# SMSD75/Timetuning

Hardware: AMD Instinct MI355X
Metric: clip-frames/sec (higher is better)
Workload: dtype f32-split(f16x3); 1 GPU; C2: dino-s16 full TimeT training step (fwd+bwd+AdamW), 4-frame 224x224 clips, 32 clips/GPU, 200 prototypes; clips_per_gpu=32, num_frames=4, num_clusters=200, global_batch=32, parallelism=dp1

## Files before the change

include/timetuning_hip.h:

```cpp
#ifndef TIMETUNING_HIP_H
#define TIMETUNING_HIP_H

#include <stddef.h>
#include <stdint.h>

#ifdef __cplusplus
extern "C" {
#endif

#define TT_OK 0
#define TT_EINVAL (-1)
#define TT_ELAUNCH (-2)
#define TT_EUNSUPPORTED (-3)

typedef void* tt_stream_t;

const char* tt_last_error(void);
int tt_abi_version(void);
int tt_set_tuning_knob(const char* name, int value);
int tt_tuning_knob_info(int index, const char** name, int* default_value, int* value);
int tt_device_info(char* name, int cap);

size_t tt_linear_ksplit_workspace_bytes(void);
int tt_linear_ksplit_workspace_init(void* workspace, size_t workspace_bytes, tt_stream_t stream);
// ... 130 lines not shown
int tt_linear_bwd_weight_planes(const void* dyT_planes, long long dyT_plane_stride, const void* xT_planes, long long xT_plane_stride,
                                int planes, float* dw, int N, int K, int Mpad, void* workspace, size_t workspace_bytes,
                                tt_stream_t stream);
size_t tt_linear_bwd_weight_planes_workspace_bytes(int N, int K, int Mpad);

int tt_label_propagate_route(int fs, int g, int K, int n_last_frames, int radius, int t);
int tt_label_propagate(const float* xn, const float* seg0, int64_t* labels, double* pmap_last, int bs, int fs, int g,
                       int D, int K, int n_last_frames, int radius, int topk, float temperature, int precision, void* workspace,
                       size_t workspace_bytes, tt_stream_t stream);
size_t tt_label_propagate_workspace_bytes(int bs, int fs, int g, int D, int K, int n_last_frames);
int tt_label_propagate_sims(const float* xn, int bs, int fs, int g, int D, int K, int n_last_frames, int precision, void* workspace,
                            size_t workspace_bytes, tt_stream_t stream);
int tt_label_propagate_from_sims(const float* xn, const float* seg0, int64_t* labels, double* pmap_last, int bs, int fs, int g, int D, int K,
                                 int n_last_frames, int radius, int topk, float temperature, void* workspace, size_t workspace_bytes,
                                 tt_stream_t stream);

int tt_label_propagate_maps(const float* xn, const float* seg0, double* pmap_all, int bs, int fs, int g, int D, int K,
                            int n_last_frames, int radius, int topk, float temperature, int precision, void* workspace,
                            size_t workspace_bytes, tt_stream_t stream);
int tt_upsample_argmax(const double* maps, int64_t* labels_out, int M, int g, int K, int R, tt_stream_t stream);
int tt_confusion_counts(const int64_t* pred, const int64_t* gt, long long n, int C, unsigned long long* counts,
                        tt_stream_t stream);

#define TT_LABELS_I16 0
#define TT_LABELS_I64 1
int tt_confusion_segments_route(int Cg, int Cp);
int tt_confusion_counts_segments(const void* pred, int pred_dtype, const int64_t* gt, int S, long long n, int Cg, int Cp, long long ignore_gt,
                                 int has_ignore, unsigned long long* counts, tt_stream_t stream);

#define TT_LABELS_U8 2
// ... 174 lines not shown
```

timetuning_amd/_lib.py:

```python
from __future__ import annotations

import ctypes as C
import os
import subprocess

_HERE = os.path.dirname(os.path.abspath(__file__))
LIB_PATH = os.environ.get("TT_LIB_PATH") or os.path.join(_HERE, "libtimetuning_hip.so")
CSRC = os.path.join(_HERE, "csrc")

c_f32p = C.c_void_p
c_vp = C.c_void_p
c_i = C.c_int
c_ll = C.c_longlong
c_f = C.c_float
c_d = C.c_double
c_sz = C.c_size_t


class AdamwTensor(C.Structure):
    _fields_ = [("p", C.c_void_p), ("g", C.c_void_p), ("m", C.c_void_p), ("v", C.c_void_p), ("n", C.c_longlong),
                ("lr", C.c_float), ("weight_decay", C.c_float)]


class VitBlockParams(C.Structure):
# ... 125 lines not shown
    "tt_kmeans_assign_route": (c_i, [c_i]),
    "tt_kmeans_accumulate": (c_i, [c_vp, c_vp, c_vp, c_vp, c_ll, c_i, c_i, c_vp, c_sz, c_vp]),
    "tt_kmeans_tiled_shape_ok": (c_i, [c_i, c_i]),
    "tt_kmeans_tile_centroids": (c_i, [c_i]),
    "tt_kmeans_assign_tiled": (c_i, [c_vp, c_vp, c_vp, c_vp, c_ll, c_i, c_i, c_i, c_vp]),
    "tt_kmeans_accumulate_tiled_workspace_bytes": (c_sz, [c_ll, c_i, c_i, c_i]),
    "tt_kmeans_accumulate_tiled": (c_i, [c_vp, c_vp, c_vp, c_vp, c_ll, c_i, c_i, c_i, c_vp, c_sz, c_vp]),
    "tt_kmeans_fit_shape_ok": (c_i, [c_ll, c_i, c_i]),
    "tt_kmeans_fit_lds_bytes": (c_sz, [c_ll, c_i, c_i]),
    "tt_kmeans_fit_workspace_bytes": (c_sz, [c_i, c_i, c_ll, c_i, c_i]),
    "tt_kmeans_fit_batched": (c_i, [c_vp, c_vp, c_vp, c_vp, c_vp, c_vp, c_i, c_ll, c_i, c_i, c_i, c_i, c_vp, c_sz, c_vp]),
    "tt_kmeans_fit_batched_split": (c_i, [c_vp, c_vp, c_vp, c_vp, c_vp, c_vp, c_i, c_ll, c_i, c_i, c_i, c_i, c_vp, c_sz, c_vp, c_i, c_vp]),
    "tt_kmeans_assign_batched": (c_i, [c_vp, c_vp, c_vp, c_vp, c_i, c_ll, c_i, c_i, c_vp]),
    "tt_label_propagate_sims": (c_i, [c_vp, c_i, c_i, c_i, c_i, c_i, c_i, c_i, c_vp, c_sz, c_vp]),
    "tt_label_propagate_from_sims": (c_i, [c_vp, c_vp, c_vp, c_vp, c_i, c_i, c_i, c_i, c_i, c_i, c_i, c_i, c_f, c_vp, c_sz, c_vp]),
    "tt_label_propagate_maps": (c_i, [c_vp, c_vp, c_vp, c_i, c_i, c_i, c_i, c_i, c_i, c_i, c_i, c_f, c_i, c_vp, c_sz, c_vp]),
    "tt_upsample_argmax": (c_i, [c_vp, c_vp, c_i, c_i, c_i, c_i, c_vp]),
    "tt_confusion_counts": (c_i, [c_vp, c_vp, c_ll, c_i, c_vp, c_vp]),
    "tt_confusion_segments_route": (c_i, [c_i, c_i]),
    "tt_confusion_counts_segments": (c_i, [c_vp, c_i, c_vp, c_i, c_ll, c_i, c_i, c_ll, c_i, c_vp, c_vp]),
    "tt_overlay_grid": (c_i, [c_vp, c_i, c_vp, C.POINTER(C.c_float), C.POINTER(C.c_float), c_vp, c_vp, c_i, c_i, c_i, c_vp, c_vp, c_vp, c_i, c_i, c_vp,
                              c_i, c_d, c_i, c_i, c_i, c_i, c_vp]),
    "tt_upsample_argmax_hist_f32": (c_i, [c_vp, c_vp, c_i, c_i, c_i, c_i, c_vp]),
    "tt_label_propagate_grid_workspace_bytes": (c_sz, [c_i, c_i, c_i, c_i, c_i, c_i, c_i, c_i]),
    "tt_label_propagate_grid_maps": (c_i, [c_vp, c_vp, c_vp, c_i, c_i, c_i, c_i, c_i, c_i, c_i, c_i, c_i, c_f, c_i, c_vp, c_sz, c_vp]),
    "tt_upsample_argmax_hw": (c_i, [c_vp, c_vp, c_i, c_i, c_i, c_i, c_i, c_i, c_vp]),
    "tt_probe_logits": (c_i, [c_vp, c_vp, c_vp, c_vp, c_ll, c_i, c_i, c_vp]),
    "tt_probe_upsample_ce_workspace_bytes": (c_sz, [c_i, c_i]),
    "tt_probe_upsample_ce": (c_i, [c_vp, c_vp, c_vp, c_vp, c_vp, c_i, c_i, c_i, c_i, c_vp, c_sz, c_vp]),
    "tt_bilinear_adjoint_tokens": (c_i, [c_vp, c_vp, c_i, c_i, c_i, c_i, c_vp]),
# ... 65 lines not shown
```

timetuning_amd/csrc/label_prop.hip:

```cpp
#include "common.hpp"

namespace tt {

int launch_gemm_plain2(const float* A, const float* B, float* C, int M, int N, int K, int lda, int ldb, int ldc, int batch_inner,
                       int batch_outer, long long sA, long long sB, long long sC, long long sA2, long long sB2, long long sC2, int bf16,
                       hipStream_t s);

constexpr int LP_MAXC = 8;
constexpr int LP_CAND_MAX = 16;

struct LpArgs {
  const float* sims;
  const float* seg0;
  const double* seg_prev;
  double* seg_out;
  int64_t* labels;
  int ctx_frame[LP_MAXC];
  int c, cs, bs, g, K, radius, topk;
  float temp;
};

template <int LP_CAND>
__global__ __launch_bounds__(256) void label_prop_kernel(LpArgs a) {
  __shared__ float s_val[4];
// ... 145 lines not shown
    s_besti[wave] = besti;
  }
  __syncthreads();
  if (tid == 0) {
    best = s_best[0];
    besti = s_besti[0];
    for (int w = 1; w < 4; ++w)
      if (s_best[w] > best || (s_best[w] == best && s_besti[w] < besti)) {
        best = s_best[w];
        besti = s_besti[w];
      }
    a.labels[(long long)b * n + qi] = besti;
  }
}

template <int CTX, int KT>
__global__ __launch_bounds__(256) void label_prop_wave_kernel(LpArgs a) {
  constexpr int CPL = 4 * CTX;
  const int lane = threadIdx.x & 63;
  const int n = a.g * a.g;
  const long long item = (long long)blockIdx.x * 4 + (threadIdx.x >> 6);
  if (item >= (long long)a.bs * n) return;
  const int b = (int)(item / n), qi = (int)(item - (long long)b * n);
  const int qy = qi / a.g, qx = qi - qy * a.g;
  const int y0 = max(0, qy - a.radius), y1 = min(a.g - 1, qy + a.radius);
  const int x0 = max(0, qx - a.radius), x1 = min(a.g - 1, qx + a.radius);
  const int ww = x1 - x0 + 1, wh = y1 - y0 + 1;
  const int total = ww * wh * a.c;
  const int lx = lane & 15, ly = lane >> 4;

  float val[CPL];
  int src[CPL];
#pragma unroll
  for (int j = 0; j < CTX; ++j) {
    const float* row = a.sims + (((long long)b * a.cs + j) * n + qi) * n;
#pragma unroll
    for (int r = 0; r < 4; ++r) {
      const int i = j * 4 + r, y = ly + 4 * r;
      val[i] = -1.f;
      src[i] = -1;
      if (j < a.c && lx < ww && y < wh) {
        const int sp = (y0 + y) * a.g + x0 + lx;
        val[i] = expf(row[sp] / a.temp);
        src[i] = (j << 12) | sp;
      }
    }
  }
  float thr = 0.f;
  unsigned taken = 0u;
  const int rounds = min(a.topk, total);
  for (int rd = 0; rd < rounds; ++rd) {
    float bv = -2.f;
    int bi = 0x7fffffff;
#pragma unroll
    for (int i = 0; i < CPL; ++i)
      if (!((taken >> i) & 1u) && src[i] >= 0 && val[i] > bv) {
        bv = val[i];
        bi = lane + 64 * i;
      }
#pragma unroll
    for (int o = 32; o > 0; o >>= 1) {
      const float ov = __shfl_xor(bv, o, 64);
      const int oi = __shfl_xor(bi, o, 64);
      if (ov > bv || (ov == bv && oi < bi)) {
        bv = ov;
        bi = oi;
      }
    }
    thr = bv;
    if ((bi & 63) == lane) taken |= 1u << (bi >> 6);
  }
  if (total < a.topk) thr = 0.f;
  float mysum = 0.f;
#pragma unroll
  for (int i = 0; i < CPL; ++i)
    if (src[i] >= 0 && val[i] >= thr) mysum += val[i];
  const float colsum = wave_sum(mysum);

  double acc[KT];
#pragma unroll
  for (int t = 0; t < KT; ++t) acc[t] = 0.0;
  const long long fstride = (long long)a.bs * n * a.K;
#pragma unroll
  for (int i = 0; i < CPL; ++i) {
    unsigned long long mask = __ballot(src[i] >= 0 && val[i] >= thr);
    while (mask) {
      const int l = __builtin_ctzll(mask);
      mask &= mask - 1;
      const int s_ = __shfl(src[i], l, 64);
      const double w = (double)(__shfl(val[i], l, 64) / colsum);
      const int fr = a.ctx_frame[s_ >> 12];
      const long long off = ((long long)b * n + (s_ & 4095)) * a.K;
#pragma unroll
      for (int t = 0; t < KT; ++t) {
        const int k = lane + 64 * t;
        if (k < a.K) acc[t] += ((fr == 0) ? (double)a.seg0[off + k] : a.seg_prev[(long long)(fr - 1) * fstride + off + k]) * w;
      }
    }
  }
  double best = -1.0;
  int besti = 0x7fffffff;
#pragma unroll
  for (int t = 0; t < KT; ++t) {
    const int k = lane + 64 * t;
    if (k < a.K) {
      a.seg_out[((long long)b * n + qi) * a.K + k] = acc[t];
      if (acc[t] > best) {
        best = acc[t];
        besti = k;
      }
    }
  }
  if (!a.labels) return;
#pragma unroll
  for (int o = 32; o > 0; o >>= 1) {
    const double ov = __shfl_xor(best, o, 64);
    const int oi = __shfl_xor(besti, o, 64);
    if (ov > best || (ov == best && oi < besti)) {
      best = ov;
      besti = oi;
    }
  }
  if (lane == 0) a.labels[(long long)b * n + qi] = besti;
}

__global__ void f64_copy_kernel(const double* __restrict__ src, double* __restrict__ dst, long long n) {
  long long i = (long long)blockIdx.x * blockDim.x + threadIdx.x;
  const long long st = (long long)gridDim.x * blockDim.x;
  for (; i < n; i += st) dst[i] = src[i];
}

static int lp_cmax(int fs, int n_last) {
  int c = 1 + (fs - 2 < n_last ? fs - 2 : n_last);
  return c < 1 ? 1 : c;
}

static int lp_route(int fs, int g, int K, int n_last, int radius, int t) {
  if (fs < 2 || g <= 0 || K <= 0 || n_last < 0 || n_last + 1 > LP_MAXC || radius <= 0 || t < 1 || t >= fs) return 0;
// ... 49 lines not shown

using namespace tt;

extern "C" size_t tt_label_propagate_workspace_bytes(int bs, int fs, int g, int D, int K, int n_last_frames) {
  (void)D;
  const size_t n = (size_t)g * g;
  return lp_workspace(lp_chunk(bs, fs, (int)n, n_last_frames), bs, fs, n, K, n_last_frames);
}

extern "C" int tt_label_propagate_route(int fs, int g, int K, int n_last_frames, int radius, int t) {
  return lp_route(fs, g, K, n_last_frames, radius, t);
}

static int lp_run(const char* who, const float* xn, const float* seg0, int64_t* labels, double* pmap_last, double* pmap_all, int bs,
                  int fs, int g, int D, int K, int n_last_frames, int radius, int topk, float temperature, int precision, void* workspace,
                  size_t workspace_bytes, tt_stream_t stream, int phase = 0) {
  TT_REQUIRE(xn && (seg0 || phase == 1) && workspace, "%s: null pointer", who);
  TT_REQUIRE(precision >= TT_PRECISION_F32 && precision <= TT_PRECISION_BF16, "%s: precision must be 0, 1 or 2 (got %d)", who, precision);
  const int sims_bf16 = precision == TT_PRECISION_BF16;
  TT_REQUIRE(bs > 0 && fs >= 2 && g > 0 && D > 0 && K > 0, "%s: need fs >= 2 and positive sizes", who);
  TT_REQUIRE(n_last_frames >= 0 && n_last_frames + 1 <= LP_MAXC, "%s: n_last_frames must be <= %d", who, LP_MAXC - 1);
  TT_REQUIRE(radius > 0, "%s: size_mask_neighborhood must be > 0 (the unrestricted variant is not built)", who);
  TT_REQUIRE(topk >= 1, "%s: topk >= 1", who);
  const int win = (2 * radius + 1 < g ? 2 * radius + 1 : g);
  const long long cand_max = (long long)win * win * lp_cmax(fs, n_last_frames);
  TT_REQUIRE(cand_max <= 256LL * LP_CAND_MAX, "%s: window %dx%d with %d context frames exceeds %d candidates per query", who, win, win,
             lp_cmax(fs, n_last_frames), 256 * LP_CAND_MAX);
  TT_REQUIRE(D % 4 == 0, "%s: feature dim must be a multiple of 4", who);
  if (lp_route(fs, g, K, n_last_frames, radius, 1) >= 5)
    TT_REQUIRE(bs <= 65535, "%s: %d clips exceed the 65535 of one launch of the workgroup-per-query kernel", who, bs);
  TT_REQUIRE(bs <= 65535, "%s: %d clips exceed the 65535 problems of one similarity launch", who, bs);
  hipStream_t s = as_stream(stream);
  const int n = g * g;
  int T = lp_chunk(bs, fs, n, n_last_frames);
  while (T > 1 && lp_workspace(T, bs, fs, (size_t)n, K, n_last_frames) > workspace_bytes) --T;
  TT_REQUIRE(workspace_bytes >= lp_workspace(T, bs, fs, (size_t)n, K, n_last_frames), "%s: workspace too small", who);
  const int cmax = lp_cmax(fs, n_last_frames);
  const size_t sims_bytes = (((size_t)T * bs * cmax * n * n * sizeof(float)) + 255) / 256 * 256;
  float* sims = static_cast<float*>(workspace);
  double* segs = pmap_all ? pmap_all : reinterpret_cast<double*>(static_cast<char*>(workspace) + sims_bytes);
  const long long fstride = (long long)bs * n * K;
  const long long per_t = (long long)bs * cmax * ((long long)n * n);
  if (phase != 0 && T < fs - 1) {
    if (phase == 1) return 1;
    set_error("%s: the similarities of %d target frames do not fit one chunk of this workspace (chunk %d)", who, fs - 1, T);
    return TT_EINVAL;
  }
  for (int t0 = 1; t0 < fs; t0 += T) {
    const int t1 = t0 + T < fs ? t0 + T : fs;
    if (phase != 2) {
      const int rc = lp_sims_chunk(xn, sims, t0, t1, bs, n, D, cmax, n_last_frames, sims_bf16, s);
      if (rc != TT_OK) return rc;
    }
    if (phase == 1) return TT_OK;
    for (int t = t0; t < t1; ++t) {
      LpArgs a{};
      int c = 0;
      a.ctx_frame[c++] = 0;
      const int lo = (t - n_last_frames > 1) ? t - n_last_frames : 1;
      for (int fr = lo; fr < t; ++fr) a.ctx_frame[c++] = fr;
      a.sims = sims + (t - t0) * per_t;
      a.seg0 = seg0;
      a.seg_prev = segs;
      a.seg_out = segs + (long long)(t - 1) * fstride;
      a.labels = (t == fs - 1) ? labels : nullptr;
      a.c = c; a.cs = cmax; a.bs = bs; a.g = g; a.K = K; a.radius = radius; a.topk = topk; a.temp = temperature;
      const unsigned wgrid = (unsigned)(((long long)bs * n + 3) / 4);
      switch (lp_route(fs, g, K, n_last_frames, radius, t)) {
        case 1: hipLaunchKernelGGL((label_prop_wave_kernel<3, 4>), dim3(wgrid), dim3(256), 0, s, a); break;
        case 2: hipLaunchKernelGGL((label_prop_wave_kernel<3, 8>), dim3(wgrid), dim3(256), 0, s, a); break;
        case 3: hipLaunchKernelGGL((label_prop_wave_kernel<8, 4>), dim3(wgrid), dim3(256), 0, s, a); break;
        case 4: hipLaunchKernelGGL((label_prop_wave_kernel<8, 8>), dim3(wgrid), dim3(256), 0, s, a); break;
        case 5: hipLaunchKernelGGL((label_prop_kernel<8>), dim3(n, bs), dim3(256), 0, s, a); break;
        case 6: hipLaunchKernelGGL((label_prop_kernel<LP_CAND_MAX>), dim3(n, bs), dim3(256), 0, s, a); break;
        default: set_error("%s: no kernel for frame %d", who, t); return TT_EINVAL;
      }
      TT_CHECK_LAUNCH(who);
    }
  }
  if (pmap_last) {
    const long long cnt = fstride;
    hipLaunchKernelGGL(f64_copy_kernel, dim3(1024), dim3(256), 0, s, segs + (long long)(fs - 2) * fstride, pmap_last, cnt);
// ... 10 lines not shown
                precision, workspace, workspace_bytes, stream);
}

extern "C" int tt_label_propagate_sims(const float* xn, int bs, int fs, int g, int D, int K, int n_last_frames, int precision, void* workspace,
                                       size_t workspace_bytes, tt_stream_t stream) {
  return lp_run("label_propagate_sims", xn, nullptr, nullptr, nullptr, nullptr, bs, fs, g, D, K, n_last_frames, 1, 1, 1.0f, precision, workspace,
                workspace_bytes, stream, 1);
}

extern "C" int tt_label_propagate_from_sims(const float* xn, const float* seg0, int64_t* labels, double* pmap_last, int bs, int fs, int g, int D,
                                            int K, int n_last_frames, int radius, int topk, float temperature, void* workspace,
                                            size_t workspace_bytes, tt_stream_t stream) {
  TT_REQUIRE(labels, "label_propagate_from_sims: null pointer");
  return lp_run("label_propagate_from_sims", xn, seg0, labels, pmap_last, nullptr, bs, fs, g, D, K, n_last_frames, radius, topk, temperature,
                TT_PRECISION_F32, workspace, workspace_bytes, stream, 2);
}

extern "C" int tt_label_propagate_maps(const float* xn, const float* seg0, double* pmap_all, int bs, int fs, int g, int D, int K,
                                       int n_last_frames, int radius, int topk, float temperature, int precision, void* workspace,
                                       size_t workspace_bytes, tt_stream_t stream) {
  TT_REQUIRE(pmap_all, "label_propagate_maps: null pointer");
  return lp_run("label_propagate_maps", xn, seg0, nullptr, nullptr, pmap_all, bs, fs, g, D, K, n_last_frames, radius, topk, temperature,
                precision, workspace, workspace_bytes, stream);
}

namespace tt {
struct LpGridArgs {
  const float* sims;
  const float* seg0;
  const double* seg_prev;
// ... 302 lines not shown
```

timetuning_amd/csrc/rowops.hip:

```cpp
#include <type_traits>

#include "common.hpp"

namespace tt {

constexpr int kMaxPerLane = 16;

template <class Out>
__global__ __launch_bounds__(256) void layernorm_fwd_kernel(const float* __restrict__ x, const float* __restrict__ gamma,
                                                            const float* __restrict__ beta, Out out, float* __restrict__ mean_out,
                                                            float* __restrict__ rstd_out, int rows, int D, float eps, int skip_group) {
  const int lane = threadIdx.x & 63;
  const int row = blockIdx.x * 4 + (threadIdx.x >> 6);
  if (row >= rows) return;
  const long long in_row = skip_group ? (long long)(row / (skip_group - 1)) * skip_group + 1 + row % (skip_group - 1) : row;
  const float* xr = x + in_row * D;
  bool bad = false;
  float v[kMaxPerLane];
  float s = 0.f;
#pragma unroll
  for (int i = 0; i < kMaxPerLane; ++i) {
    const int c = lane + 64 * i;
    v[i] = (c < D) ? xr[c] : 0.f;
    s += v[i];
// ... 454 lines not shown
  for (long long i = (long long)blockIdx.x * 256 + threadIdx.x; i < t.n; i += (long long)gridDim.x * 256) {
    const float g = t.g[i];
    float p = t.p[i] * decay;
    float m = t.m[i];
    m = m + (g - m) * (1.0f - beta1);
    const float v = t.v[i] * beta2 + (1.0f - beta2) * g * g;
    const float denom = sqrtf(v) / bc2_sqrt + eps;
    p -= step_size * (m / denom);
    t.p[i] = p;
    t.m[i] = m;
    t.v[i] = v;
  }
}

__global__ __launch_bounds__(256) void scale_tensors_kernel(AdamTable tab, const float* __restrict__ scale) {
  const tt_adamw_tensor t = tab.t[blockIdx.y];
  const float sc = *scale;
  float* gp = const_cast<float*>(t.g);
  for (long long i = (long long)blockIdx.x * 256 + threadIdx.x; i < t.n; i += (long long)gridDim.x * 256) gp[i] *= sc;
}

__global__ __launch_bounds__(256) void ema_kernel(float* __restrict__ t, const float* __restrict__ s, long long n, float m,
                                                  float one_minus_m) {
  long long i = ((long long)blockIdx.x * 256 + threadIdx.x) * 4;
  const long long stride = (long long)gridDim.x * 256 * 4;
  for (; i + 3 < n; i += stride) {
    float4 a = *reinterpret_cast<float4*>(t + i);
    const float4 b = *reinterpret_cast<const float4*>(s + i);
    a.x = a.x * one_minus_m + b.x * m;
    a.y = a.y * one_minus_m + b.y * m;
    a.z = a.z * one_minus_m + b.z * m;
    a.w = a.w * one_minus_m + b.w * m;
    *reinterpret_cast<float4*>(t + i) = a;
  }
// ... 191 lines not shown
  hipLaunchKernelGGL(adamw_kernel, dim3((unsigned)bx, count), dim3(256), 0, as_stream(stream), tab, beta1, beta2, eps, (float)bc1,
                     (float)sqrt(bc2));
  TT_CHECK_LAUNCH("adamw");
  return TT_OK;
}

extern "C" int tt_scale_tensors(const tt_adamw_tensor* tensors, int count, const float* scale_device, tt_stream_t stream) {
  TT_REQUIRE(tensors && scale_device && count > 0 && count <= TT_MAX_TENSORS, "scale_tensors: need 1..%d tensors", TT_MAX_TENSORS);
  AdamTable tab{};
  long long maxn = 0;
  for (int i = 0; i < count; ++i) {
    TT_REQUIRE(tensors[i].g && tensors[i].n > 0, "scale_tensors: tensor %d has a null gradient pointer", i);
    tab.t[i] = tensors[i];
    if (tensors[i].n > maxn) maxn = tensors[i].n;
  }
  long long bx = (maxn + 255) / 256;
  if (bx > 1024) bx = 1024;
  hipLaunchKernelGGL(scale_tensors_kernel, dim3((unsigned)bx, count), dim3(256), 0, as_stream(stream), tab, scale_device);
  TT_CHECK_LAUNCH("scale_tensors");
  return TT_OK;
}

extern "C" int tt_ema_update(float* teacher, const float* student, long long n, double momentum, tt_stream_t stream) {
  TT_REQUIRE(teacher && student && n > 0, "ema: bad arguments");
  TT_REQUIRE(aligned16(teacher) && aligned16(student), "ema: buffers must be 16-byte aligned");
  long long blocks = (n / 4 + 255) / 256;
  if (blocks > 2048) blocks = 2048;
  if (blocks < 1) blocks = 1;
  hipLaunchKernelGGL(ema_kernel, dim3((unsigned)blocks), dim3(256), 0, as_stream(stream), teacher, student, n, (float)momentum,
                     (float)(1.0 - momentum));
  TT_CHECK_LAUNCH("ema");
  return TT_OK;
// ... 17 lines not shown
```

timetuning_amd/engine.py:

```python
from __future__ import annotations

from typing import Dict, List, Optional

import torch

from . import hip_ops as ops

f32 = torch.float32



def _param_tag(w: torch.Tensor, kind) -> tuple:
    static = getattr(w, "_tt_static", False) and not w.requires_grad
    return (w.data_ptr(), w._version, 0 if static else ops.PARAM_EPOCH, kind)


def weight_planes(w: torch.nn.Parameter, planes: int) -> torch.Tensor:
    hit = getattr(w, "_tt_planes", None)
    tag = _param_tag(w, planes)
    if hit is None or hit[0] != tag:
        hit = (tag, ops.split_pairs(w.detach()) if planes == 2 else ops.split_planes(w.detach(), planes))
        w._tt_planes = hit
    return hit[1]

# ... 280 lines not shown
    if planes == 1 and pos is not None:
        wp = patch_weight_planes(pe)
        keep.append(wp)
        vp.patch_wp = wp.data_ptr()
    elif planes == 2 and PATCH_PAIRS and pos is not None and pe.weight[0].numel() % 32 == 0:
        wp = patch_weight_pairs(pe)
        keep.append(wp)
        vp.patch_wp = wp.data_ptr()
    keep.append(pos)
    return vp, keep


TWO_STREAMS = __import__("os").environ.get("TT_SINGLE_STREAM") != "1"
TWO_STREAMS_MIN_FRAMES = int(__import__("os").environ.get("TT_TWO_STREAMS_MIN_FRAMES", "64"))
LP_SIMS_ON_SIDE = __import__("os").environ.get("TT_LP_SIMS_SIDE", "1") != "0"
_SIDE_STREAMS: Dict[tuple, "torch.cuda.Stream"] = {}
_SIDE_PRIORITIES = [int(v) for v in __import__("os").environ["TT_SIDE_PRIORITIES"].split(":")] if __import__("os").environ.get("TT_SIDE_PRIORITIES") else None


def side_stream(device, which: int = 0) -> "torch.cuda.Stream":
    idx = torch.device(device).index
    idx = torch.cuda.current_device() if idx is None else idx
    if _SIDE_PRIORITIES is None and which >= 2:
        which = 0
    s = _SIDE_STREAMS.get((idx, which))
    if s is None:
        prio = _SIDE_PRIORITIES[which] if _SIDE_PRIORITIES is not None else 0
        s = _SIDE_STREAMS[(idx, which)] = torch.cuda.Stream(device=idx, priority=prio)
    return s

# ... 472 lines not shown
```

timetuning_amd/hip_ops.py:

```python
from __future__ import annotations

import contextlib
import ctypes as C
import os
from typing import Optional, Sequence

import numpy as np
import torch

from . import _lib

f32 = torch.float32


def _stream() -> int:
    return torch.cuda.current_stream().cuda_stream


def _p(t: Optional[torch.Tensor]):
    return None if t is None else t.data_ptr()


def _chk(t: torch.Tensor, name: str, dtype=f32) -> torch.Tensor:
    if not t.is_cuda:
# ... 547 lines not shown


def sinkhorn_from_q(Q, iters: int, row0: int = 0, rows_out: Optional[int] = None, transposed: bool = False):
    lib = _lib.load()
    _chk(Q, "Q")
    B, K = Q.shape if transposed else Q.shape[::-1]
    rows_out = B - row0 if rows_out is None else rows_out
    q = torch.empty((rows_out, K), dtype=f32, device=Q.device)
    nb = lib.tt_sinkhorn_workspace_bytes(B, K)
    ws = _ws(nb, Q.device)
    _lib.check(lib.tt_sinkhorn_from_q(_p(Q), int(transposed), _p(q), B, K, row0, rows_out, int(iters), _p(ws), nb, _stream()),
               "tt_sinkhorn_from_q")
    return q


def label_propagate_sims(xn, K: int, n_last_frames=7):
    lib = _lib.load()
    _chk(xn, "xn")
    fs, bs, n, D = xn.shape
    g = int(round(n ** 0.5))
    assert g * g == n
    nb = lib.tt_label_propagate_workspace_bytes(bs, fs, g, D, K, n_last_frames)
    ws = _ws(nb, xn.device)
    rc = lib.tt_label_propagate_sims(_p(xn), bs, fs, g, D, K, n_last_frames, precision_code(), _p(ws), nb, _stream())
    if rc == 1:
        return None
    _lib.check(rc, "tt_label_propagate_sims")
    return ws


def label_propagate(xn, seg0, n_last_frames=7, radius=6, topk=5, temperature=0.1, return_pmap=False, sims=None):
    lib = _lib.load()
    _chk(xn, "xn"); _chk(seg0, "seg0")
    fs, bs, n, D = xn.shape
    K = seg0.shape[-1]
    g = int(round(n ** 0.5))
    assert g * g == n
    labels = torch.empty((bs, n), dtype=torch.int64, device=xn.device)
    pmap = torch.empty((bs, n, K), dtype=torch.float64, device=xn.device) if return_pmap else None
    nb = lib.tt_label_propagate_workspace_bytes(bs, fs, g, D, K, n_last_frames)
    if sims is not None:
        assert sims.numel() >= nb, (sims.numel(), nb)
        _lib.check(lib.tt_label_propagate_from_sims(_p(xn), _p(seg0), _p(labels), _p(pmap), bs, fs, g, D, K, n_last_frames, radius, topk,
                                                    float(temperature), _p(sims), sims.numel(), _stream()), "tt_label_propagate_from_sims")
        return (labels, pmap) if return_pmap else labels
    ws = _ws(nb, xn.device)
    _lib.check(lib.tt_label_propagate(_p(xn), _p(seg0), _p(labels), _p(pmap), bs, fs, g, D, K, n_last_frames, radius, topk,
                                      float(temperature), precision_code(), _p(ws), nb, _stream()), "tt_label_propagate")
    return (labels, pmap) if return_pmap else labels


def label_propagate_maps(xn, seg0, n_last_frames=7, radius=6, topk=5, temperature=0.1):
# ... 1368 lines not shown
```

timetuning_amd/time_tuning.py:

```python
from __future__ import annotations

import argparse
import copy
import os
from typing import Dict, Optional

import numpy as np
import torch
import torch.nn as nn
import torch.nn.functional as F

from . import engine
from . import hip_ops as ops
from .models import DistributedDataParallelModel, FeatureExtractor
from .my_utils import cosine_scheduler
from .visualization import localize_clip, make_overlayed_grid

world_size = 1


class PatchPrototypeSimilarity(nn.Module):

    def __init__(self, owner: "TimeT", epsilon: float = 0.05, sinkhorn_iterations: int = 10):
        super().__init__()
# ... 493 lines not shown
            ops.layernorm_fwd(tok_hi, vit.norm.weight, vit.norm.bias, drop_first_token=True, out=feats[f0 * n:])
        xn_bb = ops.l2norm_fwd(feats).view(fs, bs, n, D)
        src_rows, tgt_rows = feats[: bs * n], feats[(fs - 1) * bs * n:]
        dbg("feats", feats); dbg("xn_bb", xn_bb)

        def target_chain():
            sv_h: Optional[dict] = {} if need_grad else None
            z_t = engine.head_forward(tgt_rows, fe.head, sv_h) if fe.head is not None else tgt_rows
            if use_mask:
                z_t = ops.scale_rows_(z_t if fe.head is not None else z_t.clone(), mask_tgt)
            sv_s: Optional[dict] = {} if need_grad else None
            return z_t, engine.prototype_scores(z_t, self.prototypes.data, sv_s), sv_h, sv_s

        tgt = None
        lp_sims = lp_ready = None
        side = engine.side_stream(dev) if engine.two_streams(dev, Fr) else None
        if side is not None:
            if fe.head is not None and engine._head_pairs_ok(engine.head_linears(fe.head), tgt_rows.shape[0]):
                for lin_ in engine.head_linears(fe.head):
                    engine.weight_planes(lin_.weight, 2)
            side.wait_stream(torch.cuda.current_stream())
            with torch.cuda.stream(side):
                lp_sims = ops.label_propagate_sims(xn_bb, self.prototypes.shape[0], hp["n_last_frames"]) if engine.LP_SIMS_ON_SIDE else None
                if lp_sims is not None:
                    lp_ready = torch.cuda.Event()
                    lp_ready.record()
                tgt = target_chain()

        if self.teacher is not None:
            tvit = self.teacher.backbone
            t_aux: Optional[dict] = {} if use_mask else None
            if "stream" in teach:
                torch.cuda.current_stream().wait_stream(teach["stream"])
                z_q = teach["z_q"]
            else:
                if tap is not None:
                    t_tok = engine.vit_blocks(tvit, tap["x"], t_first, last_block_aux=t_aux)
                    if use_mask and t_first == depth:
                        t_aux["qkv"] = qkv_src
# ... 26 lines not shown
        if self.queue_is_full():
            scores_q = torch.empty((z_q.shape[0] + self.queue.shape[0], protos_q.shape[0]), dtype=torch.float32, device=dev)
            engine.prototype_scores(z_q, protos_q, out=scores_q[: z_q.shape[0]])
            engine.prototype_scores(self.queue, protos_q, out=scores_q[z_q.shape[0]:])
        else:
            scores_q = engine.prototype_scores(z_q, protos_q)
        dbg("z_q", z_q); dbg("scores_q", scores_q)
        gather = engine.global_sinkhorn_begin(scores_q)

        if side is None:
            tgt = target_chain()
        K = self.prototypes.shape[0]
        q = engine.global_sinkhorn_end(gather, bs * n, hp["epsilon"], hp["iters"])
        if lp_ready is not None:
            torch.cuda.current_stream().wait_event(lp_ready)
        labels = ops.label_propagate(xn_bb, q.view(bs, n, K), hp["n_last_frames"], hp["radius"], hp["topk"], 0.1, sims=lp_sims)
        if side is not None:
            torch.cuda.current_stream().wait_stream(side)
        z_tgt, scores_t, sv_head, sv_sc = tgt
        ce_labels = labels
        if hp.get("target_labels") is not None:
            ce_labels = torch.as_tensor(hp["target_labels"]).to(device=dev, dtype=torch.int64).reshape(bs, n).contiguous()
        loss, dscores = ops.ce_loss_fwd_bwd(scores_t, ce_labels.view(-1), 0.1, need_grad, row_weight=mask_tgt)
        dbg("z_tgt", z_tgt); dbg("scores_t", scores_t); dbg("q", q); dbg("labels", labels); dbg("loss", loss); dbg("dscores", dscores)
        self.last_aux = dict(q=q.view(bs, n, K), target_scores=scores_t.view(bs, n, K), labels=labels)
        if use_mask:
            self.last_aux.update(target_mask=mask_tgt.view(bs, n), source_mask=mask_q.view(bs, n))
        if not need_grad:
            return loss, {}

        grads: Dict[nn.Parameter, torch.Tensor] = {}
# ... 483 lines not shown
```

Before: 19170 clip-frames/sec.

## Precompute label-propagation top-k selection lists on side stream; vectorize grad scaling

Splits label propagation into a selection pass that runs on the side stream right after the similarity computation and writes compact per-query (source, weight) lists, plus an apply pass on the main stream that only gathers segment rows from those lists. This takes the top-k selection off the critical path after Sinkhorn, since it only depends on features and not on the assignments. Queries with more than 16 kept entries fall back to the full select-and-accumulate path. Separately, the gradient scale kernel now exits early when the scale is 1 and uses float4 accesses with a smaller grid.

```diff
diff --git a/include/timetuning_hip.h b/include/timetuning_hip.h
--- a/include/timetuning_hip.h
+++ b/include/timetuning_hip.h
@@ -168,6 +168,12 @@
 int tt_label_propagate_from_sims(const float* xn, const float* seg0, int64_t* labels, double* pmap_last, int bs, int fs, int g, int D, int K,
                                  int n_last_frames, int radius, int topk, float temperature, void* workspace, size_t workspace_bytes,
                                  tt_stream_t stream);
+size_t tt_label_propagate_select_workspace_bytes(int bs, int fs, int g, int D, int K, int n_last_frames, size_t* list_offset);
+int tt_label_propagate_select(const float* xn, int bs, int fs, int g, int D, int K, int n_last_frames, int radius, int topk,
+                              float temperature, void* workspace, size_t workspace_bytes, int* overflow_count, tt_stream_t stream);
+int tt_label_propagate_from_selection(const float* xn, const float* seg0, int64_t* labels, double* pmap_last, double* pmap_all, int bs, int fs,
+                                      int g, int D, int K, int n_last_frames, int radius, int topk, float temperature, void* workspace,
+                                      size_t workspace_bytes, int* overflow_count, tt_stream_t stream);
 
 int tt_label_propagate_maps(const float* xn, const float* seg0, double* pmap_all, int bs, int fs, int g, int D, int K,
                             int n_last_frames, int radius, int topk, float temperature, int precision, void* workspace,
diff --git a/timetuning_amd/_lib.py b/timetuning_amd/_lib.py
--- a/timetuning_amd/_lib.py
+++ b/timetuning_amd/_lib.py
@@ -163,6 +163,10 @@
     "tt_kmeans_assign_batched": (c_i, [c_vp, c_vp, c_vp, c_vp, c_i, c_ll, c_i, c_i, c_vp]),
     "tt_label_propagate_sims": (c_i, [c_vp, c_i, c_i, c_i, c_i, c_i, c_i, c_i, c_vp, c_sz, c_vp]),
     "tt_label_propagate_from_sims": (c_i, [c_vp, c_vp, c_vp, c_vp, c_i, c_i, c_i, c_i, c_i, c_i, c_i, c_i, c_f, c_vp, c_sz, c_vp]),
+    "tt_label_propagate_select_workspace_bytes": (c_sz, [c_i, c_i, c_i, c_i, c_i, c_i, C.POINTER(c_sz)]),
+    "tt_label_propagate_select": (c_i, [c_vp, c_i, c_i, c_i, c_i, c_i, c_i, c_i, c_i, c_f, c_vp, c_sz, c_vp, c_vp]),
+    "tt_label_propagate_from_selection": (c_i, [c_vp, c_vp, c_vp, c_vp, c_vp, c_i, c_i, c_i, c_i, c_i, c_i, c_i, c_i, c_f, c_vp, c_sz, c_vp,
+                                                c_vp]),
     "tt_label_propagate_maps": (c_i, [c_vp, c_vp, c_vp, c_i, c_i, c_i, c_i, c_i, c_i, c_i, c_i, c_f, c_i, c_vp, c_sz, c_vp]),
     "tt_upsample_argmax": (c_i, [c_vp, c_vp, c_i, c_i, c_i, c_i, c_vp]),
     "tt_confusion_counts": (c_i, [c_vp, c_vp, c_ll, c_i, c_vp, c_vp]),
diff --git a/timetuning_amd/csrc/label_prop.hip b/timetuning_amd/csrc/label_prop.hip
--- a/timetuning_amd/csrc/label_prop.hip
+++ b/timetuning_amd/csrc/label_prop.hip
@@ -183,14 +183,18 @@
   }
 }
 
-template <int CTX, int KT>
-__global__ __launch_bounds__(256) void label_prop_wave_kernel(LpArgs a) {
+
+struct LpSel {
+  const float* sims;
+  int c, cs, g, radius, topk;
+  float temp;
+};
+
+template <int CTX>
+__device__ __forceinline__ void lp_select(const LpSel& a, int b, int qi, int lane, float (&val)[4 * CTX], int (&src)[4 * CTX], float& thr,
+                                          float& colsum) {
   constexpr int CPL = 4 * CTX;
-  const int lane = threadIdx.x & 63;
   const int n = a.g * a.g;
-  const long long item = (long long)blockIdx.x * 4 + (threadIdx.x >> 6);
-  if (item >= (long long)a.bs * n) return;
-  const int b = (int)(item / n), qi = (int)(item - (long long)b * n);
   const int qy = qi / a.g, qx = qi - qy * a.g;
   const int y0 = max(0, qy - a.radius), y1 = min(a.g - 1, qy + a.radius);
   const int x0 = max(0, qx - a.radius), x1 = min(a.g - 1, qx + a.radius);
@@ -198,8 +202,6 @@
   const int total = ww * wh * a.c;
   const int lx = lane & 15, ly = lane >> 4;
 
-  float val[CPL];
-  int src[CPL];
 #pragma unroll
   for (int j = 0; j < CTX; ++j) {
     const float* row = a.sims + (((long long)b * a.cs + j) * n + qi) * n;
@@ -215,7 +217,7 @@
       }
     }
   }
-  float thr = 0.f;
+  thr = 0.f;
   unsigned taken = 0u;
   const int rounds = min(a.topk, total);
   for (int rd = 0; rd < rounds; ++rd) {
@@ -244,29 +246,46 @@
 #pragma unroll
   for (int i = 0; i < CPL; ++i)
     if (src[i] >= 0 && val[i] >= thr) mysum += val[i];
-  const float colsum = wave_sum(mysum);
-
-  double acc[KT];
-#pragma unroll
-  for (int t = 0; t < KT; ++t) acc[t] = 0.0;
+  colsum = wave_sum(mysum);
+}
+
+__device__ __forceinline__ float lp_weight(float val, float colsum) { return val / colsum; }
+
+template <int KT>
+__device__ __forceinline__ void lp_accumulate(const LpArgs& a, int b, int lane, int s_, float q, double (&acc)[KT]) {
+  const int n = a.g * a.g;
   const long long fstride = (long long)a.bs * n * a.K;
+  const double w = (double)q;
+  const int fr = a.ctx_frame[s_ >> 12];
+  const long long off = ((long long)b * n + (s_ & 4095)) * a.K;
+#pragma unroll
+  for (int t = 0; t < KT; ++t) {
+    const int k = lane + 64 * t;
+    if (k < a.K) acc[t] += ((fr == 0) ? (double)a.seg0[off + k] : a.seg_prev[(long long)(fr - 1) * fstride + off + k]) * w;
+  }
+}
+
+template <int CTX, int KT>
+__device__ __forceinline__ void lp_select_accumulate(const LpArgs& a, int b, int qi, int lane, double (&acc)[KT]) {
+  constexpr int CPL = 4 * CTX;
+  float val[CPL], thr, colsum;
+  int src[CPL];
+  const LpSel sel{a.sims, a.c, a.cs, a.g, a.radius, a.topk, a.temp};
+  lp_select<CTX>(sel, b, qi, lane, val, src, thr, colsum);
 #pragma unroll
   for (int i = 0; i < CPL; ++i) {
     unsigned long long mask = __ballot(src[i] >= 0 && val[i] >= thr);
     while (mask) {
       const int l = __builtin_ctzll(mask);
       mask &= mask - 1;
-      const int s_ = __shfl(src[i], l, 64);
-      const double w = (double)(__shfl(val[i], l, 64) / colsum);
-      const int fr = a.ctx_frame[s_ >> 12];
-      const long long off = ((long long)b * n + (s_ & 4095)) * a.K;
-#pragma unroll
-      for (int t = 0; t < KT; ++t) {
-        const int k = lane + 64 * t;
-        if (k < a.K) acc[t] += ((fr == 0) ? (double)a.seg0[off + k] : a.seg_prev[(long long)(fr - 1) * fstride + off + k]) * w;
-      }
-    }
-  }
+      lp_accumulate<KT>(a, b, lane, __shfl(src[i], l, 64), lp_weight(__shfl(val[i], l, 64), colsum), acc);
+    }
+  }
+}
+
+template <int KT>
+__device__ __forceinline__ void lp_store(const LpArgs& a, int b, int qi, int lane, const double (&acc)[KT]) {
+  const int n = a.g * a.g;
   double best = -1.0;
   int besti = 0x7fffffff;
 #pragma unroll
@@ -291,6 +310,99 @@
     }
   }
   if (lane == 0) a.labels[(long long)b * n + qi] = besti;
+}
+
+template <int CTX, int KT>
+__global__ __launch_bounds__(256) void label_prop_wave_kernel(LpArgs a) {
+  const int lane = threadIdx.x & 63;
+  const int n = a.g * a.g;
+  const long long item = (long long)blockIdx.x * 4 + (threadIdx.x >> 6);
+  if (item >= (long long)a.bs * n) return;
+  const int b = (int)(item / n), qi = (int)(item - (long long)b * n);
+  double acc[KT];
+#pragma unroll
+  for (int t = 0; t < KT; ++t) acc[t] = 0.0;
+  lp_select_accumulate<CTX, KT>(a, b, qi, lane, acc);
+  lp_store<KT>(a, b, qi, lane, acc);
+}
+
+constexpr int LP_LIST_CAP = 16;
+constexpr int LP_LIST_OVERFLOW = -1;
+struct LpLists {
+  int* count;
+  int2* ent;
+};
+static size_t lp_list_count_bytes(size_t queries) { return (queries * sizeof(int) + 255) / 256 * 256; }
+static size_t lp_list_bytes(size_t queries) { return lp_list_count_bytes(queries) + queries * LP_LIST_CAP * sizeof(int2); }
+
+struct LpSelectArgs {
+  LpSel sel;
+  long long per_t;
+  LpLists out;
+  int* overflow;
+  int bs, t_first, nt, n_last;
+};
+
+template <int CTX>
+__global__ __launch_bounds__(256) void lp_select_wave_kernel(LpSelectArgs a) {
+  constexpr int CPL = 4 * CTX;
+  const int lane = threadIdx.x & 63;
+  const int n = a.sel.g * a.sel.g;
+  const long long per_frame = (long long)a.bs * n;
+  const long long item = (long long)blockIdx.x * 4 + (threadIdx.x >> 6);
+  if (item >= per_frame * a.nt) return;
+  const int f = (int)(item / per_frame);
+  const long long bq = item - f * per_frame;
+  const int b = (int)(bq / n), qi = (int)(bq - (long long)b * n);
+  const int t = a.t_first + f;
+  LpSel sel = a.sel;
+  sel.sims += f * a.per_t;
+  sel.c = 1 + (t - 1 < a.n_last ? t - 1 : a.n_last);
+  float val[CPL], thr, colsum;
+  int src[CPL];
+  lp_select<CTX>(sel, b, qi, lane, val, src, thr, colsum);
+  int kept = 0;
+#pragma unroll
+  for (int i = 0; i < CPL; ++i) kept += __popcll(__ballot(src[i] >= 0 && val[i] >= thr));
+  if (kept > LP_LIST_CAP) {
+    if (lane == 0) {
+      a.out.count[item] = LP_LIST_OVERFLOW;
+      if (a.overflow) atomicAdd(a.overflow, 1);
+    }
+    return;
+  }
+  int2* ent = a.out.ent + item * LP_LIST_CAP;
+  int pos = 0;
+#pragma unroll
+  for (int i = 0; i < CPL; ++i) {
+    const bool keep = src[i] >= 0 && val[i] >= thr;
+    const unsigned long long mask = __ballot(keep);
+    if (keep) ent[pos + __popcll(mask & ((1ull << lane) - 1ull))] = make_int2(src[i], __float_as_int(lp_weight(val[i], colsum)));
+    pos += __popcll(mask);
+  }
+  if (lane == 0) a.out.count[item] = kept;
+}
+
+template <int CTX, int KT>
+__global__ __launch_bounds__(256) void lp_apply_wave_kernel(LpArgs a, const int* __restrict__ count, const int2* __restrict__ ent,
+                                                            int* overflow) {
+  const int lane = threadIdx.x & 63;
+  const int n = a.g * a.g;
+  const long long item = (long long)blockIdx.x * 4 + (threadIdx.x >> 6);
+  if (item >= (long long)a.bs * n) return;
+  const int b = (int)(item / n), qi = (int)(item - (long long)b * n);
+  double acc[KT];
+#pragma unroll
+  for (int t = 0; t < KT; ++t) acc[t] = 0.0;
+  const int kept = count[item];
+  const int2 mine = lane < LP_LIST_CAP ? ent[item * LP_LIST_CAP + lane] : make_int2(0, 0);
+  if (kept < 0 || kept > LP_LIST_CAP) {
+    lp_select_accumulate<CTX, KT>(a, b, qi, lane, acc);
+    if (overflow && lane == 0) atomicAdd(overflow, 1);
+  } else {
+    for (int e = 0; e < kept; ++e) lp_accumulate<KT>(a, b, lane, __shfl(mine.x, e, 64), __int_as_float(__shfl(mine.y, e, 64)), acc);
+  }
+  lp_store<KT>(a, b, qi, lane, acc);
 }
 
 __global__ void f64_copy_kernel(const double* __restrict__ src, double* __restrict__ dst, long long n) {
@@ -370,8 +482,8 @@
 
 static int lp_run(const char* who, const float* xn, const float* seg0, int64_t* labels, double* pmap_last, double* pmap_all, int bs,
                   int fs, int g, int D, int K, int n_last_frames, int radius, int topk, float temperature, int precision, void* workspace,
-                  size_t workspace_bytes, tt_stream_t stream, int phase = 0) {
-  TT_REQUIRE(xn && (seg0 || phase == 1) && workspace, "%s: null pointer", who);
+                  size_t workspace_bytes, tt_stream_t stream, int phase = 0, int* overflow = nullptr) {
+  TT_REQUIRE(xn && (seg0 || phase == 1 || phase == 3) && workspace, "%s: null pointer", who);
   TT_REQUIRE(precision >= TT_PRECISION_F32 && precision <= TT_PRECISION_BF16, "%s: precision must be 0, 1 or 2 (got %d)", who, precision);
   const int sims_bf16 = precision == TT_PRECISION_BF16;
   TT_REQUIRE(bs > 0 && fs >= 2 && g > 0 && D > 0 && K > 0, "%s: need fs >= 2 and positive sizes", who);
@@ -398,13 +510,46 @@
   const long long fstride = (long long)bs * n * K;
   const long long per_t = (long long)bs * cmax * ((long long)n * n);
   if (phase != 0 && T < fs - 1) {
-    if (phase == 1) return 1;
+    if (phase != 2) return 1;
     set_error("%s: the similarities of %d target frames do not fit one chunk of this workspace (chunk %d)", who, fs - 1, T);
     return TT_EINVAL;
   }
+  LpLists lists{};
+  if (phase >= 3) {
+    const int route1 = lp_route(fs, g, K, n_last_frames, radius, 1);
+    if (route1 < 1 || route1 > 4) return 1;
+    const size_t queries = (size_t)(fs - 1) * bs * n;
+    const size_t list_off = (lp_workspace(T, bs, fs, (size_t)n, K, n_last_frames) + 255) / 256 * 256;
+    TT_REQUIRE(workspace_bytes >= list_off + lp_list_bytes(queries), "%s: workspace without the list region (%zu bytes, need %zu)", who,
+               workspace_bytes, list_off + lp_list_bytes(queries));
+    TT_REQUIRE(queries <= 0x7fffffffULL, "%s: %zu queries exceed one launch", who, queries);
+    lists.count = reinterpret_cast<int*>(static_cast<char*>(workspace) + list_off);
+    lists.ent = reinterpret_cast<int2*>(static_cast<char*>(workspace) + list_off + lp_list_count_bytes(queries));
+  }
+  if (phase == 3) {
+    const int t_mid = n_last_frames <= 2 ? fs : (fs < 4 ? fs : 4);
+    for (int part = 0; part < 2; ++part) {
+      const int ta = part == 0 ? 1 : t_mid, tb = part == 0 ? t_mid : fs;
+      if (tb <= ta) continue;
+      LpSelectArgs sa{};
+      sa.sel = LpSel{sims + (ta - 1) * per_t, 0, cmax, g, radius, topk, temperature};
+      sa.per_t = per_t;
+      sa.out.count = lists.count + (long long)(ta - 1) * bs * n;
+      sa.out.ent = lists.ent + (long long)(ta - 1) * bs * n * LP_LIST_CAP;
+      sa.overflow = overflow;
+      sa.bs = bs; sa.t_first = ta; sa.nt = tb - ta; sa.n_last = n_last_frames;
+      const unsigned sgrid = (unsigned)(((long long)(tb - ta) * bs * n + 3) / 4);
+      if (part == 0)
+        hipLaunchKernelGGL((lp_select_wave_kernel<3>), dim3(sgrid), dim3(256), 0, s, sa);
+      else
+        hipLaunchKernelGGL((lp_select_wave_kernel<8>), dim3(sgrid), dim3(256), 0, s, sa);
+      TT_CHECK_LAUNCH(who);
+    }
+    return TT_OK;
+  }
   for (int t0 = 1; t0 < fs; t0 += T) {
     const int t1 = t0 + T < fs ? t0 + T : fs;
-    if (phase != 2) {
+    if (phase != 2 && phase != 4) {
       const int rc = lp_sims_chunk(xn, sims, t0, t1, bs, n, D, cmax, n_last_frames, sims_bf16, s);
       if (rc != TT_OK) return rc;
     }
@@ -422,6 +567,19 @@
       a.labels = (t == fs - 1) ? labels : nullptr;
       a.c = c; a.cs = cmax; a.bs = bs; a.g = g; a.K = K; a.radius = radius; a.topk = topk; a.temp = temperature;
       const unsigned wgrid = (unsigned)(((long long)bs * n + 3) / 4);
+      if (phase == 4) {
+        const int* cnt = lists.count + (long long)(t - 1) * bs * n;
+        const int2* ent = lists.ent + (long long)(t - 1) * bs * n * LP_LIST_CAP;
+        switch (lp_route(fs, g, K, n_last_frames, radius, t)) {
+          case 1: hipLaunchKernelGGL((lp_apply_wave_kernel<3, 4>), dim3(wgrid), dim3(256), 0, s, a, cnt, ent, overflow); break;
+          case 2: hipLaunchKernelGGL((lp_apply_wave_kernel<3, 8>), dim3(wgrid), dim3(256), 0, s, a, cnt, ent, overflow); break;
+          case 3: hipLaunchKernelGGL((lp_apply_wave_kernel<8, 4>), dim3(wgrid), dim3(256), 0, s, a, cnt, ent, overflow); break;
+          case 4: hipLaunchKernelGGL((lp_apply_wave_kernel<8, 8>), dim3(wgrid), dim3(256), 0, s, a, cnt, ent, overflow); break;
+          default: set_error("%s: no list kernel for frame %d", who, t); return TT_EINVAL;
+        }
+        TT_CHECK_LAUNCH(who);
+        continue;
+      }
       switch (lp_route(fs, g, K, n_last_frames, radius, t)) {
         case 1: hipLaunchKernelGGL((label_prop_wave_kernel<3, 4>), dim3(wgrid), dim3(256), 0, s, a); break;
         case 2: hipLaunchKernelGGL((label_prop_wave_kernel<3, 8>), dim3(wgrid), dim3(256), 0, s, a); break;
@@ -462,6 +620,30 @@
   TT_REQUIRE(labels, "label_propagate_from_sims: null pointer");
   return lp_run("label_propagate_from_sims", xn, seg0, labels, pmap_last, nullptr, bs, fs, g, D, K, n_last_frames, radius, topk, temperature,
                 TT_PRECISION_F32, workspace, workspace_bytes, stream, 2);
+}
+
+extern "C" size_t tt_label_propagate_select_workspace_bytes(int bs, int fs, int g, int D, int K, int n_last_frames, size_t* list_offset) {
+  (void)D;
+  if (list_offset) *list_offset = 0;
+  if (bs <= 0 || fs < 2 || g <= 0 || K <= 0 || n_last_frames < 0) return 0;
+  const size_t n = (size_t)g * g;
+  const size_t off = (lp_workspace(lp_chunk(bs, fs, (int)n, n_last_frames), bs, fs, n, K, n_last_frames) + 255) / 256 * 256;
+  if (list_offset) *list_offset = off;
+  return off + lp_list_bytes((size_t)(fs - 1) * bs * n);
+}
+
+extern "C" int tt_label_propagate_select(const float* xn, int bs, int fs, int g, int D, int K, int n_last_frames, int radius, int topk,
+                                         float temperature, void* workspace, size_t workspace_bytes, int* overflow_count, tt_stream_t stream) {
+  return lp_run("label_propagate_select", xn, nullptr, nullptr, nullptr, nullptr, bs, fs, g, D, K, n_last_frames, radius, topk, temperature,
+                TT_PRECISION_F32, workspace, workspace_bytes, stream, 3, overflow_count);
+}
+
+extern "C" int tt_label_propagate_from_selection(const float* xn, const float* seg0, int64_t* labels, double* pmap_last, double* pmap_all, int bs,
+                                                 int fs, int g, int D, int K, int n_last_frames, int radius, int topk, float temperature,
+                                                 void* workspace, size_t workspace_bytes, int* overflow_count, tt_stream_t stream) {
+  TT_REQUIRE(labels || pmap_last || pmap_all, "label_propagate_from_selection: no output");
+  return lp_run("label_propagate_from_selection", xn, seg0, labels, pmap_last, pmap_all, bs, fs, g, D, K, n_last_frames, radius, topk,
+                temperature, TT_PRECISION_F32, workspace, workspace_bytes, stream, 4, overflow_count);
 }
 
 extern "C" int tt_label_propagate_maps(const float* xn, const float* seg0, double* pmap_all, int bs, int fs, int g, int D, int K,
diff --git a/timetuning_amd/csrc/rowops.hip b/timetuning_amd/csrc/rowops.hip
--- a/timetuning_amd/csrc/rowops.hip
+++ b/timetuning_amd/csrc/rowops.hip
@@ -492,10 +492,25 @@
 }
 
 __global__ __launch_bounds__(256) void scale_tensors_kernel(AdamTable tab, const float* __restrict__ scale) {
+  const float sc = *scale;
+  if (sc == 1.0f) return;
   const tt_adamw_tensor t = tab.t[blockIdx.y];
-  const float sc = *scale;
   float* gp = const_cast<float*>(t.g);
-  for (long long i = (long long)blockIdx.x * 256 + threadIdx.x; i < t.n; i += (long long)gridDim.x * 256) gp[i] *= sc;
+  const long long tid = (long long)blockIdx.x * 256 + threadIdx.x, stride = (long long)gridDim.x * 256;
+  long long head = (long long)(((16u - (unsigned)(reinterpret_cast<uintptr_t>(gp) & 15u)) & 15u) >> 2);
+  if (head > t.n) head = t.n;
+  const long long nvec = (t.n - head) >> 2, tail = head + 4 * nvec;
+  float4* vp = reinterpret_cast<float4*>(gp + head);
+  for (long long i = tid; i < nvec; i += stride) {
+    float4 v = vp[i];
+    v.x *= sc;
+    v.y *= sc;
+    v.z *= sc;
+    v.w *= sc;
+    vp[i] = v;
+  }
+  const long long rest = head + (t.n - tail);
+  for (long long i = tid; i < rest; i += stride) gp[i < head ? i : tail + (i - head)] *= sc;
 }
 
 __global__ __launch_bounds__(256) void ema_kernel(float* __restrict__ t, const float* __restrict__ s, long long n, float m,
@@ -717,8 +732,9 @@
     tab.t[i] = tensors[i];
     if (tensors[i].n > maxn) maxn = tensors[i].n;
   }
-  long long bx = (maxn + 255) / 256;
-  if (bx > 1024) bx = 1024;
+  long long bx = (maxn / 4 + 255) / 256;
+  if (bx > 256) bx = 256;
+  if (bx < 1) bx = 1;
   hipLaunchKernelGGL(scale_tensors_kernel, dim3((unsigned)bx, count), dim3(256), 0, as_stream(stream), tab, scale_device);
   TT_CHECK_LAUNCH("scale_tensors");
   return TT_OK;
diff --git a/timetuning_amd/engine.py b/timetuning_amd/engine.py
--- a/timetuning_amd/engine.py
+++ b/timetuning_amd/engine.py
@@ -318,6 +318,7 @@
 TWO_STREAMS = __import__("os").environ.get("TT_SINGLE_STREAM") != "1"
 TWO_STREAMS_MIN_FRAMES = int(__import__("os").environ.get("TT_TWO_STREAMS_MIN_FRAMES", "64"))
 LP_SIMS_ON_SIDE = __import__("os").environ.get("TT_LP_SIMS_SIDE", "1") != "0"
+LP_SELECT_ON_SIDE = __import__("os").environ.get("TT_LP_SELECT_SIDE", "1") != "0"
 _SIDE_STREAMS: Dict[tuple, "torch.cuda.Stream"] = {}
 _SIDE_PRIORITIES = [int(v) for v in __import__("os").environ["TT_SIDE_PRIORITIES"].split(":")] if __import__("os").environ.get("TT_SIDE_PRIORITIES") else None
 
diff --git a/timetuning_amd/hip_ops.py b/timetuning_amd/hip_ops.py
--- a/timetuning_amd/hip_ops.py
+++ b/timetuning_amd/hip_ops.py
@@ -585,14 +585,14 @@
     return q
 
 
-def label_propagate_sims(xn, K: int, n_last_frames=7):
+def label_propagate_sims(xn, K: int, n_last_frames=7, with_lists=False):
     lib = _lib.load()
     _chk(xn, "xn")
     fs, bs, n, D = xn.shape
     g = int(round(n ** 0.5))
     assert g * g == n
     nb = lib.tt_label_propagate_workspace_bytes(bs, fs, g, D, K, n_last_frames)
-    ws = _ws(nb, xn.device)
+    ws = _ws(lib.tt_label_propagate_select_workspace_bytes(bs, fs, g, D, K, n_last_frames, None) if with_lists else nb, xn.device)
     rc = lib.tt_label_propagate_sims(_p(xn), bs, fs, g, D, K, n_last_frames, precision_code(), _p(ws), nb, _stream())
     if rc == 1:
         return None
@@ -600,13 +600,48 @@
     return ws
 
 
-def label_propagate(xn, seg0, n_last_frames=7, radius=6, topk=5, temperature=0.1, return_pmap=False, sims=None):
+def label_propagate_select(xn, sims, K: int, n_last_frames=7, radius=6, topk=5, temperature=0.1, overflow=None) -> bool:
+    lib = _lib.load()
+    _chk(xn, "xn")
+    fs, bs, n, D = xn.shape
+    g = int(round(n ** 0.5))
+    assert g * g == n
+    rc = lib.tt_label_propagate_select(_p(xn), bs, fs, g, D, K, n_last_frames, radius, topk, float(temperature), _p(sims), sims.numel(),
+                                       _p(overflow), _stream())
+    if rc == 1:
+        return False
+    _lib.check(rc, "tt_label_propagate_select")
+    return True
+
+
+def label_propagate_from_selection(xn, seg0, sims, n_last_frames=7, radius=6, topk=5, temperature=0.1, return_maps=False, overflow=None):
     lib = _lib.load()
     _chk(xn, "xn"); _chk(seg0, "seg0")
     fs, bs, n, D = xn.shape
     K = seg0.shape[-1]
     g = int(round(n ** 0.5))
     assert g * g == n
+    labels = torch.empty((bs, n), dtype=torch.int64, device=xn.device)
+    maps = torch.empty((fs - 1, bs, n, K), dtype=torch.float64, device=xn.device) if return_maps else None
+    rc = lib.tt_label_propagate_from_selection(_p(xn), _p(seg0), _p(labels), None, _p(maps), bs, fs, g, D, K, n_last_frames, radius, topk,
+                                               float(temperature), _p(sims), sims.numel(), _p(overflow), _stream())
+    if rc == 1:
+        return None
+    _lib.check(rc, "tt_label_propagate_from_selection")
+    return (labels, maps) if return_maps else labels
+
+
+def label_propagate(xn, seg0, n_last_frames=7, radius=6, topk=5, temperature=0.1, return_pmap=False, sims=None, selected=False):
+    lib = _lib.load()
+    _chk(xn, "xn"); _chk(seg0, "seg0")
+    fs, bs, n, D = xn.shape
+    K = seg0.shape[-1]
+    g = int(round(n ** 0.5))
+    assert g * g == n
+    if selected and sims is not None and not return_pmap:
+        labels = label_propagate_from_selection(xn, seg0, sims, n_last_frames, radius, topk, temperature)
+        if labels is not None:
+            return labels
     labels = torch.empty((bs, n), dtype=torch.int64, device=xn.device)
     pmap = torch.empty((bs, n, K), dtype=torch.float64, device=xn.device) if return_pmap else None
     nb = lib.tt_label_propagate_workspace_bytes(bs, fs, g, D, K, n_last_frames)
diff --git a/timetuning_amd/time_tuning.py b/timetuning_amd/time_tuning.py
--- a/timetuning_amd/time_tuning.py
+++ b/timetuning_amd/time_tuning.py
@@ -531,6 +531,7 @@
 
         tgt = None
         lp_sims = lp_ready = None
+        lp_selected = False
         side = engine.side_stream(dev) if engine.two_streams(dev, Fr) else None
         if side is not None:
             if fe.head is not None and engine._head_pairs_ok(engine.head_linears(fe.head), tgt_rows.shape[0]):
@@ -538,8 +539,12 @@
                     engine.weight_planes(lin_.weight, 2)
             side.wait_stream(torch.cuda.current_stream())
             with torch.cuda.stream(side):
-                lp_sims = ops.label_propagate_sims(xn_bb, self.prototypes.shape[0], hp["n_last_frames"]) if engine.LP_SIMS_ON_SIDE else None
+                lp_sel = engine.LP_SELECT_ON_SIDE
+                lp_sims = (ops.label_propagate_sims(xn_bb, self.prototypes.shape[0], hp["n_last_frames"], with_lists=lp_sel)
+                           if engine.LP_SIMS_ON_SIDE else None)
                 if lp_sims is not None:
+                    lp_selected = lp_sel and ops.label_propagate_select(xn_bb, lp_sims, self.prototypes.shape[0], hp["n_last_frames"],
+                                                                        hp["radius"], hp["topk"], 0.1)
                     lp_ready = torch.cuda.Event()
                     lp_ready.record()
                 tgt = target_chain()
@@ -596,7 +601,7 @@
         q = engine.global_sinkhorn_end(gather, bs * n, hp["epsilon"], hp["iters"])
         if lp_ready is not None:
             torch.cuda.current_stream().wait_event(lp_ready)
-        labels = ops.label_propagate(xn_bb, q.view(bs, n, K), hp["n_last_frames"], hp["radius"], hp["topk"], 0.1, sims=lp_sims)
+        labels = ops.label_propagate(xn_bb, q.view(bs, n, K), hp["n_last_frames"], hp["radius"], hp["topk"], 0.1, sims=lp_sims, selected=lp_selected)
         if side is not None:
             torch.cuda.current_stream().wait_stream(side)
         z_tgt, scores_t, sv_head, sv_sc = tgt
```

Result: no change. 19170 clip-frames/sec, median of 2 (-0.0%).
